# HpWang-whu/YOHO

Hardware: AMD Instinct MI355X
Metric: keypoints/sec (5000 kp x60 rot desc+YOHO-O) (higher is better)
Workload: dtype fp16x2 split (2^-22-accurate products, fp32 accumulate); 1 GPU

## Files before the change

yoho_amd/csrc/gemmf.h:

```cpp
#pragma once
#include <hip/hip_runtime.h>
#include <type_traits>
#include "common.h"

namespace yoho {

typedef float floatx16 __attribute__((ext_vector_type(16)));
typedef float floatx4 __attribute__((ext_vector_type(4)));
typedef unsigned uintx4 __attribute__((ext_vector_type(4)));
typedef _Float16 halfx8 __attribute__((ext_vector_type(8)));
typedef const __attribute__((address_space(1))) void* gptr_t;
typedef __attribute__((address_space(3))) void* lptr_t;

constexpr int FG_STAGE = 32768;
constexpr int FG_LDS = 4 * FG_STAGE;

static const int FG_ORD_D[NIR_ORD] = {5, 4, 3, 3, 1};
static const int FG_ORD_R[NIR_ORD] = {4, 3, 1, 2, 0};
static const int FG_IR_BASE[5] = {0, 1, 10, 19, 35};
static const int FG_IR_D[5] = {1, 3, 3, 4, 5};

struct FGemmArgs {
    const char* A;
    const char* B;
    const float* bias;
    const float* res;
    float* out;
    long long a_off[NIR_ORD], b_off[NIR_ORD];
    int NT[NIR_ORD], MT[NIR_ORD], rot[NIR_ORD];
    int dim[NIR_ORD], qbase[NIR_ORD];
    int cin, cout, kppad, nT32;
    float descale;
    int* rflag;
    const unsigned* amax;
};

template <int I, int N, typename Fn>
__device__ __forceinline__ void sfor(Fn&& f) {
    if constexpr (I < N) {
        f(std::integral_constant<int, I>{});
        sfor<I + 1, N>(f);
    }
}

__device__ __forceinline__ floatx16 mfma_h(uintx4 a, uintx4 b, floatx16 c) {
    union { uintx4 u; halfx8 h; } ca, cb;
    ca.u = a; cb.u = b;
    return __builtin_amdgcn_mfma_f32_32x32x16_f16(ca.h, cb.h, c, 0, 0, 0);
}

__device__ __forceinline__ const char* uniform_ptr(const char* p) {
    const unsigned long long v = reinterpret_cast<unsigned long long>(p);
    const unsigned lo = __builtin_amdgcn_readfirstlane((unsigned)v), hi = __builtin_amdgcn_readfirstlane((unsigned)(v >> 32));
    return reinterpret_cast<const char*>(((unsigned long long)hi << 32) | lo);
}

template <int MI, int NJ>
__device__ __forceinline__ void zero_acc(floatx16 (&acc)[MI][NJ]) {
#pragma unroll
    for (int i = 0; i < MI; ++i)
#pragma unroll
        for (int j = 0; j < NJ; ++j)
#pragma unroll
            for (int e = 0; e < 16; ++e) acc[i][j][e] = 0.f;
}

__device__ __forceinline__ bool fg3_map(const FGemmArgs& a, int xcd, int slot, int& t, int& local, int& r) {
    int start = 0;
    for (int u = 0; u < NIR_ORD; ++u) {
        const int ru = (xcd + a.rot[u]) & 7;
        const int cnt = a.NT[u] > ru ? ((a.NT[u] - 1 - ru) / 8 + 1) * a.MT[u] : 0;
        if (slot < start + cnt) { t = u; local = slot - start; r = ru; return true; }
        start += cnt;
    }
    return false;
}

inline int fgemm_grid(const FGemmArgs& a, int per_tile) {
    int tot = 0;
    for (int x = 0; x < 8; ++x) {
        int n = 0;
        for (int t = 0; t < NIR_ORD; ++t) {
            const int r = (x + a.rot[t]) & 7;
            if (a.NT[t] > r) n += ((a.NT[t] - 1 - r) / 8 + 1) * a.MT[t] * per_tile;
        }
        tot = n > tot ? n : tot;
    }
    return 8 * tot;
}

enum { F2_NOSTORE = 0x100, F2_MIX = 0x200, F2_ST_SC1 = 0x400, F2_ST_NT = 0x800, F2_SPARSE4 = 0x1000, F2_SPARSE16 = 0x2000 };

__device__ __forceinline__ size_t slab_off(int tile32, int q, int cout8, int o, int half, int kp32) {
    return (((((size_t)tile32 * G + q) * cout8 + (o >> 3)) * 2 + half) * TILE + kp32) * 4;
}

template <int MI, int NJ>
__device__ __forceinline__ void residual_start(floatx16 (&acc)[MI][NJ], int row0, int kp0, int jidx, int d, int qbase, const float* res, float descale,
                                               int cout, int nT32, int lane) {
    const float inv = 1.f / descale;
    const int half = lane >> 5, kp32 = lane & 31, cout8 = cout >> 3;
#pragma unroll
    for (int bi = 0; bi < NJ; ++bi) {
        const int tile32 = (kp0 >> 5) + bi;
#pragma unroll
        for (int ai = 0; ai < MI; ++ai) {
            const int rowb = row0 + ai * 32;
            const int iidx = rowb / cout, o0 = rowb - iidx * cout;
            const bool ok = tile32 < nT32 && iidx < d;
            const int q = qbase + iidx * d + jidx;
#pragma unroll
            for (int q4 = 0; q4 < 4; ++q4) {
                const size_t off = slab_off(tile32, q, cout8, o0 + q4 * 8 + half * 4, half, kp32);
                const floatx4 v = *reinterpret_cast<const floatx4*>(res + (ok ? off : 0)) * (ok ? inv : 0.f);
                acc[ai][bi][4 * q4 + 0] = v.x; acc[ai][bi][4 * q4 + 1] = v.y;
                acc[ai][bi][4 * q4 + 2] = v.z; acc[ai][bi][4 * q4 + 3] = v.w;
            }
        }
    }
}

template <int MI, int NJ>
__device__ __forceinline__ void coef_epilogue(const floatx16 (&acc)[MI][NJ], int row0, int kp0, int jidx, int d, int qbase, float* out, const float* bias,
                                              float descale, int cout, int nT32, int* rflag, int lane, int flags) {
    const int half = lane >> 5, kp32 = lane & 31, cout8 = cout >> 3;
    unsigned top = 0u;
#ifdef YOHO_EXPERIMENTS
    if ((flags & F2_SPARSE4) && (blockIdx.x >> 3) % 4 != 0) flags |= F2_NOSTORE;
    if ((flags & F2_SPARSE16) && (blockIdx.x >> 3) % 16 != 0) flags |= F2_NOSTORE;
    const __amdgpu_buffer_rsrc_t orsrc = __builtin_amdgcn_make_buffer_rsrc(out, 0, 0x7FFFFFFF, 0x00020000);
#endif
#pragma unroll
    for (int bi = 0; bi < NJ; ++bi) {
        const int tile32 = (kp0 >> 5) + bi;
        if (tile32 >= nT32) continue;
#pragma unroll
        for (int ai = 0; ai < MI; ++ai) {
            const int rowb = row0 + ai * 32;
            const int iidx = rowb / cout, o0 = rowb - iidx * cout;
            if (iidx >= d) continue;
            const int q = qbase + iidx * d + jidx;
#pragma unroll
            for (int q4 = 0; q4 < 4; ++q4) {
                const int o = o0 + q4 * 8 + half * 4;
                floatx4 val;
                val.x = acc[ai][bi][4 * q4 + 0]; val.y = acc[ai][bi][4 * q4 + 1];
                val.z = acc[ai][bi][4 * q4 + 2]; val.w = acc[ai][bi][4 * q4 + 3];
                val *= descale;
                if (d == 1) val += *reinterpret_cast<const floatx4*>(bias + o) * 7.745966692414834f;
                const size_t off = slab_off(tile32, q, cout8, o, half, kp32);
#ifdef YOHO_EXPERIMENTS
                if (flags & F2_ST_SC1) __builtin_amdgcn_raw_buffer_store_b128(__builtin_bit_cast(uintx4, val), orsrc, (int)(off * 4), 0, 16);
                else if (flags & F2_ST_NT) __builtin_amdgcn_raw_buffer_store_b128(__builtin_bit_cast(uintx4, val), orsrc, (int)(off * 4), 0, 2);
                else if (!(flags & F2_NOSTORE))
#endif
                *reinterpret_cast<floatx4*>(out + off) = val;
                top = max(max(top, __float_as_uint(val.x) & 0x7FFFFFFFu), __float_as_uint(val.y) & 0x7FFFFFFFu);
                top = max(max(top, __float_as_uint(val.z) & 0x7FFFFFFFu), __float_as_uint(val.w) & 0x7FFFFFFFu);
            }
        }
    }
    note_range_bits(rflag, top, FP16_MAX / HF_ASCALE);
}

void fgemm_fill_args(FGemmArgs& a, const Layer& L, const char* Bplanes, int kppad, int nT32, const float* res, float* out, int* rflag);
int launch_fgemm2(const FGemmArgs& a, int flags, hipStream_t s);
int launch_fgemm3(const FGemmArgs& a, int flags, hipStream_t s);
int fgemm2_init();

}
```

yoho_amd/csrc/gemmf.hip:

```cpp
#include <hip/hip_runtime.h>
#include <hip/hip_fp16.h>
#include <type_traits>
#include <vector>
#include <cmath>
#include <cstring>
#include <cstdlib>

#include "common.h"
#include "gemmf.h"

namespace yoho {

struct Frags {
    uintx4 ah[4], al[4], bh[4], bl[4];
};

template <int SUB, int R>
__device__ __forceinline__ void read_frag(const char* pa, const char* pb, Frags& f) {
    constexpr int t = R & 3;
    if constexpr (R < 4) f.al[t] = *reinterpret_cast<const uintx4*>(pa + (2 + SUB) * 8192 + t * 512);
    else if constexpr (R < 8) f.bh[t] = *reinterpret_cast<const uintx4*>(pb + (0 + SUB) * 8192 + t * 512);
    else if constexpr (R < 12) f.ah[t] = *reinterpret_cast<const uintx4*>(pa + (0 + SUB) * 8192 + t * 512);
    else f.bl[t] = *reinterpret_cast<const uintx4*>(pb + (2 + SUB) * 8192 + t * 512);
}
// ... 28 lines not shown
        acc[g >> 2][g & 3] = mfma_h(f.al[g >> 2], f.bh[g & 3], acc[g >> 2][g & 3]);
        read_frag<RSUB, g>(ra, rb, nf);
        __builtin_amdgcn_sched_barrier(0);
    });
    sfor<0, 16>([&](auto gc) {
        constexpr int g = decltype(gc)::value;
        acc[g >> 2][g & 3] = mfma_h(f.ah[g >> 2], f.bl[g & 3], acc[g >> 2][g & 3]);
        if constexpr (DMA) {
            stage_unit<g>(srcA, srcB, dmadst, w, lane16);
            __builtin_amdgcn_sched_barrier(0);
        }
    });
    __builtin_amdgcn_sched_barrier(0);
    sfor<0, 16>([&](auto gc) {
        constexpr int g = decltype(gc)::value;
        acc[g >> 2][g & 3] = mfma_h(f.ah[g >> 2], f.bh[g & 3], acc[g >> 2][g & 3]);
    });
    __builtin_amdgcn_sched_barrier(0);
}

__global__ __launch_bounds__(256, 1) void fgemm_kernel(FGemmArgs a, int flags) {
    extern __shared__ __attribute__((aligned(16))) char smem[];
    const int tid = threadIdx.x, lane = tid & 63;
    const int w = __builtin_amdgcn_readfirstlane(tid >> 6);
    int t = 0, local = 0, r = 0;
    if (!fg3_map(a, blockIdx.x & 7, blockIdx.x >> 3, t, local, r)) return;
    const int d = a.dim[t];
    const int MT = a.MT[t], KS = d * a.cin / 32;
    const int cg = local / MT, mtile = local - cg * MT;
    const int ntile = r + 8 * cg;
    const char* Ag = a.A + a.a_off[t] + (size_t)mtile * KS * FG_STAGE;
    const char* Bg = a.B + a.b_off[t] + (size_t)ntile * KS * FG_STAGE;
    const int wm = w >> 1, wn = w & 1;
    const int lane16 = lane * 16;
    const int row0 = mtile * 256 + wm * 128;
    const int col0 = ntile * 256 + wn * 128;

    floatx16 acc[4][4];
    zero_acc(acc);

    const int lane_a = (lane >> 5) * 4096 + (wm * 128 + (lane & 31)) * 16;
    const int lane_b = FG_STAGE + (lane >> 5) * 4096 + (wn * 128 + (lane & 31)) * 16;

    stage_tile(Ag, smem, w, lane);
    stage_tile(Bg, smem + FG_STAGE, w, lane);
    if (KS > 1) {
        stage_tile(Ag + FG_STAGE, smem + 2 * FG_STAGE, w, lane);
        stage_tile(Bg + FG_STAGE, smem + 3 * FG_STAGE, w, lane);
    }
    if ((flags & EPI_RES) && row0 < d * a.cout) residual_start(acc, row0, col0 % a.kppad, col0 / a.kppad, d, a.qbase[t], a.res, a.descale, a.cout, a.nT32, lane);
    asm volatile("s_waitcnt vmcnt(0)" ::: "memory");
    __syncthreads();

    if (row0 >= d * a.cout) {
        for (int s = 0; s < KS; ++s) {
            asm volatile("s_waitcnt vmcnt(0)" ::: "memory");
            __syncthreads();
            const int s2 = s + 2 < KS ? s + 2 : KS - 1;
            char* cur = smem + (s & 1) * (2 * FG_STAGE);
            stage_tile(Ag + (size_t)s2 * FG_STAGE, cur, w, lane);
            stage_tile(Bg + (size_t)s2 * FG_STAGE, cur + FG_STAGE, w, lane);
        }
        asm volatile("s_waitcnt vmcnt(0)" ::: "memory");
        return;
    }
    Frags P, Q;
    read_frags<0>(smem + lane_a, smem + lane_b, P);
    for (int s = 0; s < KS; ++s) {
        char* cur = smem + (s & 1) * (2 * FG_STAGE);
        char* nxt = smem + ((s + 1) & 1) * (2 * FG_STAGE);
        substep<1, false>(P, acc, cur + lane_a, cur + lane_b, Q, nullptr, nullptr, nullptr, w, lane16);
        asm volatile("s_waitcnt vmcnt(0) lgkmcnt(0)" ::: "memory");
        __syncthreads();
        __builtin_amdgcn_sched_barrier(0);
        const int s2 = s + 2 < KS ? s + 2 : KS - 1;
        substep<0, true>(Q, acc, nxt + lane_a, nxt + lane_b, P, uniform_ptr(Ag + (size_t)s2 * FG_STAGE), uniform_ptr(Bg + (size_t)s2 * FG_STAGE),
                              cur, w, lane16);
    }
    asm volatile("s_waitcnt vmcnt(0)" ::: "memory");

    coef_epilogue(acc, row0, col0 % a.kppad, col0 / a.kppad, d, a.qbase[t], a.out, a.bias, a.descale, a.cout, a.nT32, a.rflag, lane, flags);
}

int fgemm_init() {
    HIPCHK(hipFuncSetAttribute(reinterpret_cast<const void*>(&fgemm_kernel), hipFuncAttributeMaxDynamicSharedMemorySize, FG_LDS));
    if (int rc = cgemm_init()) return rc;
    return fgemm2_init();
}

static long long pack_off(int t, int rows, int kdim) {
    long long off = 0;
    for (int u = 0; u < t; ++u) off += (long long)((FG_ORD_D[u] * rows + 255) / 256) * (FG_ORD_D[u] * kdim / 32) * FG_STAGE;
    return off;
}

size_t fgemm_planes_bytes(int kppad, int cin) { return (size_t)pack_off(NIR_ORD, kppad, cin); }

void fgemm_qinfo(int* qi ) {
    for (int t = 0; t < NIR_ORD; ++t) {
        const int r = FG_ORD_R[t], d = FG_IR_D[r];
        for (int m = 0; m < d; ++m)
            for (int j = 0; j < d; ++j) {
                int* p = qi + (FG_IR_BASE[r] + m * d + j) * 4;
                p[0] = t; p[1] = m; p[2] = j; p[3] = d;
            }
    }
}
void fgemm_plane_offsets(int kppad, int cin, long long* off ) {
    for (int t = 0; t < NIR_ORD; ++t) off[t] = pack_off(t, kppad, cin);
}

static inline unsigned short half_bits_h(float x) {
    const _Float16 h = (_Float16)x;
    unsigned short u;
    std::memcpy(&u, &h, 2);
    return u;
}

static unsigned char e4m3_bits(float x) {
    const unsigned sgn = std::signbit(x) ? 0x80u : 0u;
    const float a = std::fabs(x);
    if (!(a == a)) return 0x7F;
    if (a >= 464.f) return (unsigned char)(sgn | 0x7E);
    if (a < std::ldexp(1.f, -6)) {
        const int r = (int)std::nearbyint(std::ldexp(a, 9));
        return (unsigned char)(sgn | (r == 8 ? 0x08 : r));
    }
    int e;
    (void)std::frexp(a, &e);
    int r = (int)std::nearbyint(std::ldexp(a, 3 - (e - 1)));
    if (r == 16) { r = 8; ++e; }
    const int E = e - 1 + 7;
    if (E > 15 || (E == 15 && r - 8 > 6)) return (unsigned char)(sgn | 0x7E);
    return (unsigned char)(sgn | (E << 3) | (r - 8));
}
static inline float half_value_h(unsigned short u) {
    _Float16 h;
    std::memcpy(&h, &u, 2);
    return (float)h;
}

static inline size_t apack_index(int row, int k, int KS) {
    const int mtile = row >> 8, rr = row & 255, ks = k >> 5, sub = (k >> 4) & 1, kg = (k >> 3) & 1, e = k & 7;
    return ((size_t)mtile * KS + ks) * (FG_STAGE / 2) + ((size_t)(sub * 2 + kg) * 256 + rr) * 8 + e;
}
static inline void put_split(unsigned short* pack, size_t idx, float x) {
    const _Float16 hi = (_Float16)x;
    pack[idx] = half_bits_h(x);
    pack[idx + 8192] = half_bits_h(x - (float)hi);
}
static void fp8_correction_planes(const std::vector<unsigned short>& out, std::vector<unsigned short>& out8) {
    out8 = out;
    const size_t nblk = out.size() / (FG_STAGE / 2);
    for (size_t b = 0; b < nblk; ++b) {
        const unsigned short* src = out.data() + b * (FG_STAGE / 2);
        unsigned char* dst = reinterpret_cast<unsigned char*>(out8.data() + b * (FG_STAGE / 2) + 8192);
        for (int u = 0; u < 1024; ++u)
            for (int e = 0; e < 8; ++e) {
                dst[u * 16 + e] = e4m3_bits(half_value_h(src[u * 8 + e]) * 0.25f);
                dst[u * 16 + 8 + e] = e4m3_bits(half_value_h(src[8192 + u * 8 + e]) * 512.f);
            }
    }
}

int pack_fgemm_weights(const FourierBasis& fb, const float* W, int cin, int cout, std::vector<unsigned short>& out, float* descale,
                       std::vector<unsigned short>* out8) {
    if ((cout % 256 && cout != 32) || cin % 32) return -1;
    std::vector<float> what((size_t)60 * cout * cin);
    std::vector<double> coef(60 * NTAP);
    for (int r = 0; r < 5; ++r) {
        const int d = FG_IR_D[r];
        for (int i = 0; i < d; ++i)
            for (int m = 0; m < d; ++m)
                for (int k = 0; k < NTAP; ++k) coef[(FG_IR_BASE[r] + i * d + m) * NTAP + k] = fb.rho[r][fb.n0[k]][m * d + i];
    }
    float wmax = 0.f;
    for (int f = 0; f < 60; ++f)
        for (int o = 0; o < cout; ++o)
            for (int c = 0; c < cin; ++c) {
                const float* wk = W + ((size_t)o * cin + c) * NTAP;
                double acc = 0.0;
                for (int k = 0; k < NTAP; ++k) acc += (double)wk[k] * coef[f * NTAP + k];
                const float v = (float)acc;
                what[((size_t)f * cout + o) * cin + c] = v;
                wmax = std::fmax(wmax, std::fabs(v));
            }
    int ex = 0;
    if (wmax > 0.f && std::isfinite(wmax)) (void)std::frexp(wmax, &ex);
    const float wscale = std::ldexp(1.f, 10 - ex);
    *descale = 1.f / (wscale * HF_ASCALE);
    out.assign((size_t)pack_off(NIR_ORD, cout, cin) / 2, 0);
    for (int t = 0; t < NIR_ORD; ++t) {
        const int r = FG_ORD_R[t], d = FG_IR_D[r];
        unsigned short* base = out.data() + pack_off(t, cout, cin) / 2;
        for (int i = 0; i < d; ++i)
            for (int o = 0; o < cout; ++o)
                for (int m = 0; m < d; ++m) {
                    const float* src = &what[((size_t)(FG_IR_BASE[r] + i * d + m) * cout + o) * cin];
                    for (int c = 0; c < cin; ++c) put_split(base, apack_index(i * cout + o, m * cin + c, d * cin / 32), src[c] * wscale);
                }
    }
    if (out8) fp8_correction_planes(out, *out8);
    return 0;
}

int pack_cgemm_weights(const float* W, int cin, int cout, int ntaps, std::vector<unsigned short>& out, float* descale, std::vector<unsigned short>& out8) {
    if (cout % 256 || cin % 32) return -1;
    float wmax = 0.f;
    for (size_t i = 0; i < (size_t)cout * cin * ntaps; ++i) wmax = std::fmax(wmax, std::fabs(W[i]));
    int ex = 0;
    if (wmax > 0.f && std::isfinite(wmax)) (void)std::frexp(wmax, &ex);
    const float wscale = std::ldexp(1.f, 10 - ex);
    *descale = 1.f / (wscale * H2_ASCALE);
    const int KS = ntaps * cin / 32;
    out.assign((size_t)(cout / 256) * KS * (FG_STAGE / 2), 0);
    for (int o = 0; o < cout; ++o)
        for (int tap = 0; tap < ntaps; ++tap)
            for (int c = 0; c < cin; ++c) put_split(out.data(), apack_index(o, tap * cin + c, KS), W[((size_t)o * cin + c) * ntaps + tap] * wscale);
    fp8_correction_planes(out, out8);
    return 0;
}

void fgemm_fill_args(FGemmArgs& a, const Layer& L, const char* Bplanes, int kppad, int nT32, const float* res, float* out, int* rflag) {
    a.rflag = rflag; a.amax = nullptr;
    a.A = reinterpret_cast<const char*>(L.wpg); a.B = Bplanes; a.bias = L.bias; a.res = res; a.out = out;
    a.cin = L.cin; a.cout = L.cout; a.kppad = kppad; a.nT32 = nT32; a.descale = L.wpg_descale;
    static const int ROT[NIR_ORD] = {0, 0, 4, 4, 2};
    for (int t = 0; t < NIR_ORD; ++t) {
        a.a_off[t] = pack_off(t, L.cout, L.cin);
        a.b_off[t] = pack_off(t, kppad, L.cin);
        a.MT[t] = (FG_ORD_D[t] * L.cout + 255) / 256;
        a.NT[t] = FG_ORD_D[t] * kppad / 256;
        a.rot[t] = ROT[t];
        a.dim[t] = FG_ORD_D[t];
        a.qbase[t] = FG_IR_BASE[FG_ORD_R[t]];
    }
}

int launch_fgemm(const Layer& L, const char* Bplanes, int kppad, int nT32, const float* res, float* out, int flags, hipStream_t s, int* rflag,
                 FGemmBlocking blocking, const unsigned* amax) {
    FGemmArgs a;
    fgemm_fill_args(a, L, Bplanes, kppad, nT32, res, out, rflag);
    static const int dbg_gemm1 = [] { const char* e = experiment_env("YOHO_PARTI_DEBUG"); return (e && std::strstr(e, "gemm1")) ? 1 : 0; }();
    if (dbg_gemm1) blocking = FG_TILE256_W4;
    if (blocking == FG_TILE256_W8 && amax && L.wpg8) { a.amax = amax; a.A = reinterpret_cast<const char*>(L.wpg8); }
    if (blocking == FG_TILE256_W8) return launch_fgemm3(a, flags, s);
    if (blocking != FG_TILE256_W4) return launch_fgemm2(a, flags, s);
    hipLaunchKernelGGL(fgemm_kernel, dim3(fgemm_grid(a, 1)), dim3(256), FG_LDS, s, a, flags);
    HIPCHK(hipGetLastError());
    return 0;
}

}
```

yoho_amd/csrc/gemmf2.hip:

```cpp
#include <hip/hip_runtime.h>
#include <cstdlib>
#include <cstring>
#include "common.h"
#include "gemmf.h"

namespace yoho {

constexpr int F2_BUF = 24576;
constexpr int F2_LDS = 3 * F2_BUF;
constexpr int F3_BUF = 32768;
constexpr int F3_LDS = 3 * F3_BUF;

struct Frags2 {
    uintx4 ah[4], al[4], bh[2], bl[2];
};

template <int LO, int R>
__device__ __forceinline__ void read_frag2(const char* pa, const char* pb, Frags2& f) {
    if constexpr (R < 4) f.al[R] = *reinterpret_cast<const uintx4*>(pa + 8192 + R * 512);
    else if constexpr (R < 6) f.bh[R - 4] = *reinterpret_cast<const uintx4*>(pb + (R - 4) * 512);
    else if constexpr (R < 10) f.ah[R - 6] = *reinterpret_cast<const uintx4*>(pa + (R - 6) * 512);
    else f.bl[R - 10] = *reinterpret_cast<const uintx4*>(pb + LO + (R - 10) * 512);
}
template <int LO>
// ... 135 lines not shown
    }
}

__global__ __launch_bounds__(256, 2) void fgemm2_kernel(FGemmArgs a, int flags) {
    extern __shared__ __attribute__((aligned(16))) char smem[];
    const int tid = threadIdx.x, lane = tid & 63;
    const int w = __builtin_amdgcn_readfirstlane(tid >> 6);
    int t = 0, local = 0, r = 0;
    if (!fg2_map(a, blockIdx.x & 7, blockIdx.x >> 3, (flags & F2_MIX) == 0, t, local, r)) return;
    const int d = a.dim[t];
    const int MT = a.MT[t], KS = d * a.cin / 32, KT = 2 * KS;
    const int nh = local & 1, pair = local >> 1;
    const int cg = pair / MT, mtile = pair - cg * MT;
    const int ntile = r + 8 * cg;
    const char* Ag = a.A + a.a_off[t] + (size_t)mtile * KS * FG_STAGE;
    const char* Bg = a.B + a.b_off[t] + (size_t)ntile * KS * FG_STAGE + nh * 2048;
    const int wm = w >> 1, wn = w & 1;
    const Dma2 dm(w, lane);
    const int lane_a = (lane >> 5) * 4096 + (wm * 128 + (lane & 31)) * 16;
    const int lane_b = 16384 + (lane >> 5) * 2048 + (wn * 64 + (lane & 31)) * 16;

    floatx16 acc[4][2];
    zero_acc(acc);
    auto dma = [&](int st, int buf) { dma_step(dm, Ag + step_off(st), Bg + step_off(st), smem + buf); };
    ring_prologue<F2_BUF>(KT, dma);
    const int row0 = mtile * 256 + wm * 128, colbase = ntile * 256 + nh * 128 + wn * 64;
    const bool rows_live = row0 < d * a.cout;
    const int jidx = colbase / a.kppad, kp0 = colbase - jidx * a.kppad, qbase = a.qbase[t];
    if ((flags & EPI_RES) && rows_live) residual_start(acc, row0, kp0, jidx, d, qbase, a.res, a.descale, a.cout, a.nT32, lane);
    asm volatile("s_waitcnt vmcnt(0)" ::: "memory");
    __builtin_amdgcn_s_barrier();
    if (!rows_live) return ring_pipelined_idle<F2_BUF>(KT, dma);

    Frags2 P;
    read_frags2<Dma2::LO>(smem + lane_a, smem + lane_b, P);
    ring_pipelined<F2_BUF, 6>(smem, Ag, Bg, KT, lane_a, lane_b, P,
        [&](auto dmac, const Frags2& f, Frags2& nf, const char* ra, const char* rb, const char* srcA, const char* srcB, char* buf) {
            step2<decltype(dmac)::value>(dm, f, acc, ra, rb, nf, srcA, srcB, buf);
        });
    coef_epilogue(acc, row0, kp0, jidx, d, qbase, a.out, a.bias, a.descale, a.cout, a.nT32, a.rflag, lane, flags);
}

struct Wave3 {
    int wm, wn, nh, lane_a, lane_b;
    Dma3 dm;
    __device__ __forceinline__ Wave3(int w8, int lane) : wm((w8 & 3) >> 1), wn(w8 & 1), nh(w8 >> 2), dm(w8, lane) {
        lane_a = (lane >> 5) * 4096 + (wm * 128 + (lane & 31)) * 16;
        lane_b = 16384 + (lane >> 5) * 4096 + (nh * 128 + wn * 64 + (lane & 31)) * 16;
    }
};

__global__ __launch_bounds__(512, 2) void fgemm3_kernel(FGemmArgs a, int flags) {
    extern __shared__ __attribute__((aligned(16))) char smem[];
    const int tid = threadIdx.x, lane = tid & 63;
    const Wave3 wv(__builtin_amdgcn_readfirstlane(tid >> 6), lane);
    int t = 0, local = 0, r = 0;
    if (!fg3_map(a, blockIdx.x & 7, blockIdx.x >> 3, t, local, r)) return;
    const int d = a.dim[t];
    const int MT = a.MT[t], KS = d * a.cin / 32, KT = 2 * KS;
    const int cg = local / MT, mtile = local - cg * MT;
    const int ntile = r + 8 * cg;
    const char* Ag = a.A + a.a_off[t] + (size_t)mtile * KS * FG_STAGE;
    const char* Bg = a.B + a.b_off[t] + (size_t)ntile * KS * FG_STAGE;

    floatx16 acc[4][2];
    zero_acc(acc);
    auto dma = [&](int st, int buf) { dma_step(wv.dm, Ag + step_off(st), Bg + step_off(st), smem + buf); };
    ring_prologue<F3_BUF>(KT, dma);
    const int row0 = mtile * 256 + wv.wm * 128, colbase = ntile * 256 + wv.nh * 128 + wv.wn * 64;
    const bool rows_live = row0 < d * a.cout;
    const int jidx = colbase / a.kppad, kp0 = colbase - jidx * a.kppad, qbase = a.qbase[t];
    if ((flags & EPI_RES) && rows_live) residual_start(acc, row0, kp0, jidx, d, qbase, a.res, a.descale, a.cout, a.nT32, lane);
    asm volatile("s_waitcnt vmcnt(0)" ::: "memory");
    __builtin_amdgcn_s_barrier();
    if (!rows_live) return ring_pipelined_idle<F3_BUF>(KT, dma);

    Frags2 P;
    read_frags2<Dma3::LO>(smem + wv.lane_a, smem + wv.lane_b, P);
    ring_pipelined<F3_BUF, 4>(smem, Ag, Bg, KT, wv.lane_a, wv.lane_b, P,
        [&](auto dmac, const Frags2& f, Frags2& nf, const char* ra, const char* rb, const char* srcA, const char* srcB, char* buf) {
            step2<decltype(dmac)::value>(wv.dm, f, acc, ra, rb, nf, srcA, srcB, buf);
        });
    coef_epilogue(acc, row0, kp0, jidx, d, qbase, a.out, a.bias, a.descale, a.cout, a.nT32, a.rflag, lane, flags);
}

typedef int intx8 __attribute__((ext_vector_type(8)));
typedef short shortx2 __attribute__((ext_vector_type(2)));
typedef _Float16 halfx2 __attribute__((ext_vector_type(2)));
struct Frags8 {
    intx8 a[4], b[2];
};
struct C8Scales {
    float ah = 4.f, al = 4.f / 2048.f, bh = 1.f, bl = 1.f;
    int mfma_b = 127;
    C8Scales() = default;
    __device__ __forceinline__ explicit C8Scales(const unsigned* amax) {
        const unsigned amax_bits = __builtin_amdgcn_readfirstlane(*amax);
        int kexp = (int)(amax_bits >> 23) - 127 - 7;
        kexp = kexp < -60 ? -60 : (kexp > 9 ? 9 : kexp);
        bh = __uint_as_float((unsigned)(kexp + 127) << 23); bl = __uint_as_float((unsigned)(kexp - 11 + 127) << 23);
        mfma_b = 127 + kexp;
    }
};
struct Int2 { int x, y; };
__device__ __forceinline__ Int2 frag_to_fp8(uintx4 f, float scale) {
    union { unsigned u; halfx2 h; } p0, p1, p2, p3;
    p0.u = f[0]; p1.u = f[1]; p2.u = f[2]; p3.u = f[3];
    shortx2 r = {0, 0}, q = {0, 0};
    r = __builtin_amdgcn_cvt_scalef32_pk_fp8_f16(r, p0.h, scale, false);
    r = __builtin_amdgcn_cvt_scalef32_pk_fp8_f16(r, p1.h, scale, true);
    q = __builtin_amdgcn_cvt_scalef32_pk_fp8_f16(q, p2.h, scale, false);
    q = __builtin_amdgcn_cvt_scalef32_pk_fp8_f16(q, p3.h, scale, true);
    Int2 o;
    __builtin_memcpy(&o.x, &r, 4);
    __builtin_memcpy(&o.y, &q, 4);
    return o;
}

template <int PAR>
__device__ __forceinline__ void step3c(const Frags2& f, floatx16 (&acc)[4][2], Frags8& c8, const C8Scales& sc) {
#pragma unroll
    for (int i = 0; i < 4; ++i)
#pragma unroll
        for (int j = 0; j < 2; ++j) acc[i][j] = mfma_h(f.ah[i], f.bh[j], acc[i][j]);
#pragma unroll
    for (int i = 0; i < 4; ++i)
#pragma unroll
        for (int e = 0; e < 4; ++e) c8.a[i][4 * PAR + e] = (int)f.al[i][e];
#pragma unroll
    for (int j = 0; j < 2; ++j) {
        const Int2 l = frag_to_fp8(f.bl[j], sc.bl), h = frag_to_fp8(f.bh[j], sc.bh);
        c8.b[j][4 * PAR] = l.x; c8.b[j][4 * PAR + 1] = l.y; c8.b[j][4 * PAR + 2] = h.x; c8.b[j][4 * PAR + 3] = h.y;
    }
    if constexpr (PAR == 1) {
#pragma unroll
        for (int i = 0; i < 4; ++i)
#pragma unroll
            for (int j = 0; j < 2; ++j)
                acc[i][j] = __builtin_amdgcn_mfma_scale_f32_32x32x64_f8f6f4(c8.a[i], c8.b[j], acc[i][j], 0, 0, 0, 127 + 2 - 11, 0, sc.mfma_b);
    }
}

template <bool FP8, typename BSrc>
__device__ __forceinline__ void ring_plain(floatx16 (&acc)[4][2], char* smem, const Wave3& wv, const char* Ag, BSrc&& bsrc, int KT, bool rows_live,
                                           const C8Scales& sc) {
    Frags8 c8;
    if constexpr (FP8) {
#pragma unroll
        for (int i = 0; i < 4; ++i)
#pragma unroll
            for (int e = 0; e < 8; ++e) c8.a[i][e] = 0;
#pragma unroll
        for (int j = 0; j < 2; ++j)
#pragma unroll
            for (int e = 0; e < 8; ++e) c8.b[j][e] = 0;
    }
    int cur = 0, stg = 2 * F3_BUF;
    int s = 0;
    auto stage = [&] {
        const int s2 = s + 2 < KT ? s + 2 : KT - 1;
        dma_step(wv.dm, uniform_ptr(Ag + step_off(s2)), uniform_ptr(bsrc(s2)), smem + stg);
    };
    auto rotate = [&] { stg = cur; cur = cur == 2 * F3_BUF ? 0 : cur + F3_BUF; ++s; };
    auto one_step = [&](auto parity) {
        asm volatile("s_waitcnt vmcnt(4) lgkmcnt(0)" ::: "memory");
        __builtin_amdgcn_s_barrier();
// ... 188 lines not shown

template <int R>
__device__ __forceinline__ void read_frag3s(const char* pa, const char* pb, Frags3s& f) {
    if constexpr (R < 5) f.al[R] = *reinterpret_cast<const uintx4*>(pa + 8192 + R * 512);
    else if constexpr (R == 5) f.bh = *reinterpret_cast<const uintx4*>(pb);
    else if constexpr (R < 11) f.ah[R - 6] = *reinterpret_cast<const uintx4*>(pa + (R - 6) * 512);
    else f.bl = *reinterpret_cast<const uintx4*>(pb + 8192);
}

template <bool DMA, int D>
__device__ __forceinline__ void step3s(const Frags3s& f, floatx16 (&acc)[5][1], const char* ra, const char* rb, Frags3s& nf,
                                       const char* srcA, const char* srcB, char* dmabuf, const Dma3& dm) {
    sfor<0, 5>([&](auto gc) {
        constexpr int g = decltype(gc)::value;
        if constexpr (g < D) acc[g][0] = mfma_h(f.al[g], f.bh, acc[g][0]);
        if constexpr (g < D) read_frag3s<g>(ra, rb, nf);
        if constexpr (g == 4) read_frag3s<5>(ra, rb, nf);
        __builtin_amdgcn_sched_barrier(0);
    });
    sfor<0, 5>([&](auto gc) {
        constexpr int g = decltype(gc)::value;
        if constexpr (g < D) acc[g][0] = mfma_h(f.ah[g], f.bl, acc[g][0]);
        if constexpr (g < D) read_frag3s<6 + g>(ra, rb, nf);
        if constexpr (g == 4) read_frag3s<11>(ra, rb, nf);
        __builtin_amdgcn_sched_barrier(0);
    });
    sfor<0, 5>([&](auto gc) {
        constexpr int g = decltype(gc)::value;
        if constexpr (g < D) acc[g][0] = mfma_h(f.ah[g], f.bh, acc[g][0]);
        if constexpr (DMA && g < 4) dm.template piece<g>(srcA, srcB, dmabuf);
        __builtin_amdgcn_sched_barrier(0);
    });
}

template <int D>
__device__ __forceinline__ void fgemm3s_kloop(floatx16 (&acc)[5][1], char* smem, const char* Ag, const char* Bg, int KT, const Dma3& dm, int lane_a, int lane_b) {
    Frags3s P;
    sfor<0, 12>([&](auto rc) {
        constexpr int R = decltype(rc)::value;
        if constexpr (R == 5 || R == 11 || (R < 5 && R < D) || (R > 5 && R < 11 && R - 6 < D)) read_frag3s<R>(smem + lane_a, smem + lane_b, P);
    });
    ring_pipelined<F3_BUF, 4>(smem, Ag, Bg, KT, lane_a, lane_b, P,
        [&](auto dmac, const Frags3s& f, Frags3s& nf, const char* ra, const char* rb, const char* srcA, const char* srcB, char* buf) {
            step3s<decltype(dmac)::value, D>(f, acc, ra, rb, nf, srcA, srcB, buf, dm);
        });
}

__global__ __launch_bounds__(512, 2) void fgemm3s_kernel(FGemmArgs a, int flags) {
    extern __shared__ __attribute__((aligned(16))) char smem[];
    const int tid = threadIdx.x, lane = tid & 63;
    const int w8 = __builtin_amdgcn_readfirstlane(tid >> 6);
    int t = 0, local = 0, r = 0;
    if (!fg3_map(a, blockIdx.x & 7, blockIdx.x >> 3, t, local, r)) return;
    const int d = a.dim[t];
    const int KS = d * a.cin / 32, KT = 2 * KS;
    const int ntile = r + 8 * local;
    const char* Ag = a.A + a.a_off[t];
    const char* Bg = a.B + a.b_off[t] + (size_t)ntile * KS * FG_STAGE;
    const Dma3 dm(w8, lane);
    const int lane_a = (lane >> 5) * 4096 + (lane & 31) * 16;
    const int lane_b = 16384 + (lane >> 5) * 4096 + (w8 * 32 + (lane & 31)) * 16;

    floatx16 acc[5][1];
    zero_acc(acc);
    ring_prologue<F3_BUF>(KT, [&](int st, int buf) { dma_step(dm, uniform_ptr(Ag + step_off(st)), uniform_ptr(Bg + step_off(st)), smem + buf); });
    asm volatile("s_waitcnt vmcnt(0)" ::: "memory");
    __builtin_amdgcn_s_barrier();

    switch (d) {
        case 1: fgemm3s_kloop<1>(acc, smem, Ag, Bg, KT, dm, lane_a, lane_b); break;
        case 3: fgemm3s_kloop<3>(acc, smem, Ag, Bg, KT, dm, lane_a, lane_b); break;
        case 4: fgemm3s_kloop<4>(acc, smem, Ag, Bg, KT, dm, lane_a, lane_b); break;
        default: fgemm3s_kloop<5>(acc, smem, Ag, Bg, KT, dm, lane_a, lane_b); break;
    }
    const int colbase = ntile * 256 + w8 * 32;
    const int jidx = colbase / a.kppad, kp0 = colbase - jidx * a.kppad;
    coef_epilogue(acc, 0, kp0, jidx, d, a.qbase[t], a.out, a.bias, a.descale, 32, a.nT32, a.rflag, lane, flags & F2_NOSTORE);
}

int fgemm3_init() {
    HIPCHK(hipFuncSetAttribute(reinterpret_cast<const void*>(&fgemm3_kernel), hipFuncAttributeMaxDynamicSharedMemorySize, F3_LDS));
    HIPCHK(hipFuncSetAttribute(reinterpret_cast<const void*>(&fgemm3s_kernel), hipFuncAttributeMaxDynamicSharedMemorySize, F3_LDS));
    HIPCHK(hipFuncSetAttribute(reinterpret_cast<const void*>(&fgemm3c_kernel), hipFuncAttributeMaxDynamicSharedMemorySize, F3_LDS));
    return 0;
}

int launch_fgemm3(const FGemmArgs& a, int flags, hipStream_t s) {
    if (const char* dbg = experiment_env("YOHO_FGEMM_DEBUG")) {
        if (std::strstr(dbg, "nostore")) flags |= F2_NOSTORE;
        if (std::strstr(dbg, "sc1")) flags |= F2_ST_SC1;
        if (std::strstr(dbg, "stnt")) flags |= F2_ST_NT;
    }
    const int tot = fgemm_grid(a, 1);
    static const bool small_ok = [] { const char* e = experiment_env("YOHO_FGEMM_DEBUG"); return !(e && std::strstr(e, "nosmall")); }();
    if (small_ok && a.cout == 32 && !(flags & EPI_RES)) hipLaunchKernelGGL(fgemm3s_kernel, dim3(tot), dim3(512), F3_LDS, s, a, flags);
    else if (a.amax) hipLaunchKernelGGL(fgemm3c_kernel, dim3(tot), dim3(512), F3_LDS, s, a, flags);
    else hipLaunchKernelGGL(fgemm3_kernel, dim3(tot), dim3(512), F3_LDS, s, a, flags);
    HIPCHK(hipGetLastError());
    return 0;
}

int fgemm2_init() {
    HIPCHK(hipFuncSetAttribute(reinterpret_cast<const void*>(&fgemm2_kernel), hipFuncAttributeMaxDynamicSharedMemorySize, F2_LDS));
    return fgemm3_init();
}

int launch_fgemm2(const FGemmArgs& a, int flags, hipStream_t s) {
    if (const char* dbg = experiment_env("YOHO_FGEMM_DEBUG")) {
        if (std::strstr(dbg, "nostore")) flags |= F2_NOSTORE;
        if (std::strstr(dbg, "mix")) flags |= F2_MIX;
        if (std::strstr(dbg, "sc1")) flags |= F2_ST_SC1;
        if (std::strstr(dbg, "nt")) flags |= F2_ST_NT;
        if (std::strstr(dbg, "sparse4")) flags |= F2_SPARSE4;
        if (std::strstr(dbg, "sparse16")) flags |= F2_SPARSE16;
    }
    hipLaunchKernelGGL(fgemm2_kernel, dim3(fgemm_grid(a, 2)), dim3(256), F2_LDS, s, a, flags);
    HIPCHK(hipGetLastError());
    return 0;
}

}
```

Before: 1.891 million keypoints/s.

## Add 16x16x32 MFMA GEMM kernel variants for wide layers

Adds new GEMM kernels for the three blocking schemes that use the 16x16x32 f16 MFMA instead of 32x32x16, with matching residual and epilogue routines that permute lanes back to the existing slab layout. They are selected automatically for layers with cin and cout of at least 256 when no fp8 amax path is active. The aim is higher MFMA throughput and different register and LDS reuse on large layers, at the cost of extra permlane swaps in the epilogue and more code paths to keep correct.

```diff
diff --git a/yoho_amd/csrc/gemmf.h b/yoho_amd/csrc/gemmf.h
--- a/yoho_amd/csrc/gemmf.h
+++ b/yoho_amd/csrc/gemmf.h
@@ -89,7 +89,7 @@
     return 8 * tot;
 }
 
-enum { F2_NOSTORE = 0x100, F2_MIX = 0x200, F2_ST_SC1 = 0x400, F2_ST_NT = 0x800, F2_SPARSE4 = 0x1000, F2_SPARSE16 = 0x2000 };
+enum { F2_NOSTORE = 0x100, F2_MIX = 0x200, F2_ST_SC1 = 0x400, F2_ST_NT = 0x800, F2_SPARSE4 = 0x1000, F2_SPARSE16 = 0x2000, F2_K32 = 0x4000 };
 
 __device__ __forceinline__ size_t slab_off(int tile32, int q, int cout8, int o, int half, int kp32) {
     return (((((size_t)tile32 * G + q) * cout8 + (o >> 3)) * 2 + half) * TILE + kp32) * 4;
@@ -163,6 +163,129 @@
     note_range_bits(rflag, top, FP16_MAX / HF_ASCALE);
 }
 
+__device__ __forceinline__ floatx4 mfma_h16(uintx4 a, uintx4 b, floatx4 c) {
+    union { uintx4 u; halfx8 h; } ca, cb;
+    ca.u = a; cb.u = b;
+    return __builtin_amdgcn_mfma_f32_16x16x32_f16(ca.h, cb.h, c, 0, 0, 0);
+}
+
+inline bool fgemm_layer_k32(const FGemmArgs& a) { return a.cin >= 256 && a.cin % 64 == 0 && a.cout >= 256; }
+
+template <int NJ, typename Extra>
+__device__ __forceinline__ void row_products32(floatx4 (&accrow)[NJ], const uintx4& al, const uintx4& ah, const uintx4 (&bh)[NJ], const uintx4 (&bl)[NJ],
+                                               Extra&& extra) {
+    sfor<0, 3 * NJ>([&](auto mc) {
+        constexpr int m = decltype(mc)::value, j = m % NJ, p = m / NJ;
+        accrow[j] = mfma_h16(p == 0 ? al : ah, p == 1 ? bl[j] : bh[j], accrow[j]);
+        __builtin_amdgcn_sched_barrier(0);
+        extra(mc);
+        __builtin_amdgcn_sched_barrier(0);
+    });
+}
+
+template <int LOB, int MI, int NJ>
+__device__ __forceinline__ void stage32_plain(floatx4 (&acc)[MI][NJ], const char* pa, const char* pb) {
+    uintx4 bh[NJ], bl[NJ], al[2], ah[2];
+#pragma unroll
+    for (int j = 0; j < NJ; ++j) {
+        bh[j] = *reinterpret_cast<const uintx4*>(pb + j * 256);
+        bl[j] = *reinterpret_cast<const uintx4*>(pb + LOB + j * 256);
+    }
+    al[0] = *reinterpret_cast<const uintx4*>(pa + 16384);
+    ah[0] = *reinterpret_cast<const uintx4*>(pa);
+    sfor<0, MI>([&](auto ic) {
+        constexpr int i = decltype(ic)::value;
+        if constexpr (i + 1 < MI) {
+            al[(i + 1) & 1] = *reinterpret_cast<const uintx4*>(pa + 16384 + (i + 1) * 256);
+            ah[(i + 1) & 1] = *reinterpret_cast<const uintx4*>(pa + (i + 1) * 256);
+        }
+        row_products32(acc[i], al[i & 1], ah[i & 1], bh, bl, [](auto) {});
+    });
+}
+
+template <int MI, int NJ>
+__device__ __forceinline__ void zero_acc(floatx4 (&acc)[MI][NJ]) {
+#pragma unroll
+    for (int i = 0; i < MI; ++i)
+#pragma unroll
+        for (int j = 0; j < NJ; ++j) acc[i][j] = floatx4{0.f, 0.f, 0.f, 0.f};
+}
+
+template <bool TO_SLAB>
+__device__ __forceinline__ void swap_rows16(floatx4& x, floatx4& y) {
+    typedef unsigned uintx2 __attribute__((ext_vector_type(2)));
+#pragma unroll
+    for (int e = 0; e < 4; ++e) {
+        uintx2 r = {__float_as_uint(x[e]), __float_as_uint(y[e])};
+        if constexpr (TO_SLAB) {
+            r = __builtin_amdgcn_permlane16_swap(r.x, r.y, false, false);
+            r = __builtin_amdgcn_permlane32_swap(r.x, r.y, false, false);
+        } else {
+            r = __builtin_amdgcn_permlane32_swap(r.x, r.y, false, false);
+            r = __builtin_amdgcn_permlane16_swap(r.x, r.y, false, false);
+        }
+        x[e] = __uint_as_float(r.x); y[e] = __uint_as_float(r.y);
+    }
+}
+
+template <int MI, int NJ>
+__device__ __forceinline__ void residual_start(floatx4 (&acc)[MI][NJ], int row0, int kp0, int jidx, int d, int qbase, const float* res, float descale,
+                                               int cout, int nT32, int lane) {
+    static_assert(NJ % 2 == 0, "pairs of 16-column tiles");
+    const float inv = 1.f / descale;
+    const int half = lane >> 5, kp32 = lane & 31, cout8 = cout >> 3;
+#pragma unroll
+    for (int bi = 0; bi < NJ; bi += 2) {
+        const int tile32 = (kp0 >> 5) + (bi >> 1);
+#pragma unroll
+        for (int ai = 0; ai < MI; ++ai) {
+            const int rowb = row0 + ai * 16;
+            const int iidx = rowb / cout, o0 = rowb - iidx * cout;
+            const bool ok = tile32 < nT32 && iidx < d;
+            const int q = qbase + iidx * d + jidx;
+            const size_t off0 = slab_off(tile32, q, cout8, o0 + half * 4, half, kp32), off1 = slab_off(tile32, q, cout8, o0 + 8 + half * 4, half, kp32);
+            acc[ai][bi] = *reinterpret_cast<const floatx4*>(res + (ok ? off0 : 0)) * (ok ? inv : 0.f);
+            acc[ai][bi + 1] = *reinterpret_cast<const floatx4*>(res + (ok ? off1 : 0)) * (ok ? inv : 0.f);
+            swap_rows16<false>(acc[ai][bi], acc[ai][bi + 1]);
+        }
+    }
+}
+
+template <int MI, int NJ>
+__device__ __forceinline__ void coef_epilogue(const floatx4 (&acc)[MI][NJ], int row0, int kp0, int jidx, int d, int qbase, float* out, const float* bias,
+                                              float descale, int cout, int nT32, int* rflag, int lane, int flags) {
+    static_assert(NJ % 2 == 0, "pairs of 16-column tiles");
+    const int half = lane >> 5, kp32 = lane & 31, cout8 = cout >> 3;
+    unsigned top = 0u;
+#pragma unroll
+    for (int bi = 0; bi < NJ; bi += 2) {
+        const int tile32 = (kp0 >> 5) + (bi >> 1);
+        if (tile32 >= nT32) continue;
+#pragma unroll
+        for (int ai = 0; ai < MI; ++ai) {
+            const int rowb = row0 + ai * 16;
+            const int iidx = rowb / cout, o0 = rowb - iidx * cout;
+            if (iidx >= d) continue;
+            const int q = qbase + iidx * d + jidx;
+            floatx4 v[2] = {acc[ai][bi], acc[ai][bi + 1]};
+            swap_rows16<true>(v[0], v[1]);
+#pragma unroll
+            for (int h8 = 0; h8 < 2; ++h8) {
+                const int o = o0 + h8 * 8 + half * 4;
+                floatx4 val = v[h8] * descale;
+                if (d == 1) val += *reinterpret_cast<const floatx4*>(bias + o) * 7.745966692414834f;
+#ifdef YOHO_EXPERIMENTS
+                if (!(flags & F2_NOSTORE))
+#endif
+                *reinterpret_cast<floatx4*>(out + slab_off(tile32, q, cout8, o, half, kp32)) = val;
+                top = max(max(top, __float_as_uint(val.x) & 0x7FFFFFFFu), __float_as_uint(val.y) & 0x7FFFFFFFu);
+                top = max(max(top, __float_as_uint(val.z) & 0x7FFFFFFFu), __float_as_uint(val.w) & 0x7FFFFFFFu);
+            }
+        }
+    }
+    note_range_bits(rflag, top, FP16_MAX / HF_ASCALE);
+}
+
 void fgemm_fill_args(FGemmArgs& a, const Layer& L, const char* Bplanes, int kppad, int nT32, const float* res, float* out, int* rflag);
 int launch_fgemm2(const FGemmArgs& a, int flags, hipStream_t s);
 int launch_fgemm3(const FGemmArgs& a, int flags, hipStream_t s);
diff --git a/yoho_amd/csrc/gemmf.hip b/yoho_amd/csrc/gemmf.hip
--- a/yoho_amd/csrc/gemmf.hip
+++ b/yoho_amd/csrc/gemmf.hip
@@ -134,8 +134,52 @@
     coef_epilogue(acc, row0, col0 % a.kppad, col0 / a.kppad, d, a.qbase[t], a.out, a.bias, a.descale, a.cout, a.nT32, a.rflag, lane, flags);
 }
 
+__global__ __launch_bounds__(256, 1) void fgemmk_kernel(FGemmArgs a, int flags) {
+    extern __shared__ __attribute__((aligned(16))) char smem[];
+    const int tid = threadIdx.x, lane = tid & 63;
+    const int w = __builtin_amdgcn_readfirstlane(tid >> 6);
+    int t = 0, local = 0, r = 0;
+    if (!fg3_map(a, blockIdx.x & 7, blockIdx.x >> 3, t, local, r)) return;
+    const int d = a.dim[t];
+    const int MT = a.MT[t], KS = d * a.cin / 32;
+    const int cg = local / MT, mtile = local - cg * MT;
+    const int ntile = r + 8 * cg;
+    const char* Ag = a.A + a.a_off[t] + (size_t)mtile * KS * FG_STAGE;
+    const char* Bg = a.B + a.b_off[t] + (size_t)ntile * KS * FG_STAGE;
+    const int wm = w >> 1, wn = w & 1;
+    const int row0 = mtile * 256 + wm * 128, col0 = ntile * 256 + wn * 128;
+    const bool rows_live = row0 < d * a.cout;
+    const int lane_a = (lane >> 4) * 4096 + (wm * 128 + (lane & 15)) * 16;
+    const int lane_b = FG_STAGE + (lane >> 4) * 4096 + (wn * 128 + (lane & 15)) * 16;
+
+    floatx4 acc[8][8];
+    zero_acc(acc);
+    stage_tile(Ag, smem, w, lane);
+    stage_tile(Bg, smem + FG_STAGE, w, lane);
+    if (KS > 1) {
+        stage_tile(Ag + FG_STAGE, smem + 2 * FG_STAGE, w, lane);
+        stage_tile(Bg + FG_STAGE, smem + 3 * FG_STAGE, w, lane);
+    }
+    if ((flags & EPI_RES) && rows_live) residual_start(acc, row0, col0 % a.kppad, col0 / a.kppad, d, a.qbase[t], a.res, a.descale, a.cout, a.nT32, lane);
+    asm volatile("s_waitcnt vmcnt(0)" ::: "memory");
+    __syncthreads();
+    for (int s = 0; s < KS; ++s) {
+        char* cur = smem + (s & 1) * (2 * FG_STAGE);
+        if (rows_live) stage32_plain<FG_STAGE / 2>(acc, cur + lane_a, cur + lane_b);
+        asm volatile("s_waitcnt vmcnt(0) lgkmcnt(0)" ::: "memory");
+        __syncthreads();
+        __builtin_amdgcn_sched_barrier(0);
+        if (s + 2 < KS) {
+            stage_tile(uniform_ptr(Ag + (size_t)(s + 2) * FG_STAGE), cur, w, lane);
+            stage_tile(uniform_ptr(Bg + (size_t)(s + 2) * FG_STAGE), cur + FG_STAGE, w, lane);
+        }
+    }
+    if (rows_live) coef_epilogue(acc, row0, col0 % a.kppad, col0 / a.kppad, d, a.qbase[t], a.out, a.bias, a.descale, a.cout, a.nT32, a.rflag, lane, flags);
+}
+
 int fgemm_init() {
     HIPCHK(hipFuncSetAttribute(reinterpret_cast<const void*>(&fgemm_kernel), hipFuncAttributeMaxDynamicSharedMemorySize, FG_LDS));
+    HIPCHK(hipFuncSetAttribute(reinterpret_cast<const void*>(&fgemmk_kernel), hipFuncAttributeMaxDynamicSharedMemorySize, FG_LDS));
     if (int rc = cgemm_init()) return rc;
     return fgemm2_init();
 }
@@ -296,9 +340,12 @@
     static const int dbg_gemm1 = [] { const char* e = experiment_env("YOHO_PARTI_DEBUG"); return (e && std::strstr(e, "gemm1")) ? 1 : 0; }();
     if (dbg_gemm1) blocking = FG_TILE256_W4;
     if (blocking == FG_TILE256_W8 && amax && L.wpg8) { a.amax = amax; a.A = reinterpret_cast<const char*>(L.wpg8); }
+    const char* dbg = experiment_env("YOHO_FGEMM_DEBUG");
+    if (fgemm_layer_k32(a) && !a.amax && !(dbg && std::strstr(dbg, "k16"))) flags |= F2_K32;
     if (blocking == FG_TILE256_W8) return launch_fgemm3(a, flags, s);
     if (blocking != FG_TILE256_W4) return launch_fgemm2(a, flags, s);
-    hipLaunchKernelGGL(fgemm_kernel, dim3(fgemm_grid(a, 1)), dim3(256), FG_LDS, s, a, flags);
+    if (flags & F2_K32) hipLaunchKernelGGL(fgemmk_kernel, dim3(fgemm_grid(a, 1)), dim3(256), FG_LDS, s, a, flags);
+    else hipLaunchKernelGGL(fgemm_kernel, dim3(fgemm_grid(a, 1)), dim3(256), FG_LDS, s, a, flags);
     HIPCHK(hipGetLastError());
     return 0;
 }
diff --git a/yoho_amd/csrc/gemmf2.hip b/yoho_amd/csrc/gemmf2.hip
--- a/yoho_amd/csrc/gemmf2.hip
+++ b/yoho_amd/csrc/gemmf2.hip
@@ -241,6 +241,173 @@
             step2<decltype(dmac)::value>(wv.dm, f, acc, ra, rb, nf, srcA, srcB, buf);
         });
     coef_epilogue(acc, row0, kp0, jidx, d, qbase, a.out, a.bias, a.descale, a.cout, a.nT32, a.rflag, lane, flags);
+}
+
+constexpr int F3K_BUF = 2 * FG_STAGE;
+constexpr int F3K_LDS = 2 * F3K_BUF;
+
+struct Dma3k {
+    static constexpr int NP = 8;
+    int la, ldst;
+    __device__ __forceinline__ Dma3k(int w8, int lane) : la(w8 * 1024 + lane * 16), ldst(w8 * 1024) {}
+    template <int U>
+    __device__ __forceinline__ void piece(const char* srcA, const char* srcB, char* buf) const {
+        constexpr int q = (U & 3) * 8192;
+        if constexpr (U < 4) __builtin_amdgcn_global_load_lds((gptr_t)(srcA + q + la), (lptr_t)(buf + q + ldst), 16, 0, 0);
+        else __builtin_amdgcn_global_load_lds((gptr_t)(srcB + q + la), (lptr_t)(buf + FG_STAGE + q + ldst), 16, 0, 0);
+    }
+};
+struct FragsA32 { uintx4 al, ah; };
+struct FragsB32 { uintx4 bh[4], bl[4]; };
+
+template <int R>
+__device__ __forceinline__ void read_open32(const char* pa, const char* pb, FragsA32& a0, FragsB32& b) {
+    if constexpr (R == 0) a0.al = *reinterpret_cast<const uintx4*>(pa + 16384);
+    else if constexpr (R < 5) b.bh[R - 1] = *reinterpret_cast<const uintx4*>(pb + (R - 1) * 256);
+    else if constexpr (R == 5) a0.ah = *reinterpret_cast<const uintx4*>(pa);
+    else b.bl[R - 6] = *reinterpret_cast<const uintx4*>(pb + 16384 + (R - 6) * 256);
+}
+
+template <bool DMA>
+__device__ __forceinline__ void step32(const Dma3k& dm, floatx4 (&acc)[8][4], FragsA32 (&fa)[2], const FragsB32& b, FragsB32& nb, const char* pa,
+                                       const char* npa, const char* npb, const char* srcA, const char* srcB, char* dmabuf) {
+    sfor<0, 7>([&](auto ic) {
+        constexpr int i = decltype(ic)::value;
+        row_products32(acc[i], fa[i & 1].al, fa[i & 1].ah, b.bh, b.bl, [&](auto mc) {
+            constexpr int m = decltype(mc)::value;
+            if constexpr (m == 1) fa[(i + 1) & 1].al = *reinterpret_cast<const uintx4*>(pa + 16384 + (i + 1) * 256);
+            if constexpr (m == 2) fa[(i + 1) & 1].ah = *reinterpret_cast<const uintx4*>(pa + (i + 1) * 256);
+        });
+    });
+    asm volatile("s_waitcnt vmcnt(0) lgkmcnt(0)" ::: "memory");
+    __builtin_amdgcn_s_barrier();
+    __builtin_amdgcn_sched_barrier(0);
+    row_products32(acc[7], fa[1].al, fa[1].ah, b.bh, b.bl, [&](auto mc) {
+        constexpr int m = decltype(mc)::value;
+        if constexpr (m < 5) {
+            read_open32<2 * m>(npa, npb, fa[0], nb);
+            read_open32<2 * m + 1>(npa, npb, fa[0], nb);
+        }
+        if constexpr (DMA && m >= 4) dm.template piece<m - 4>(srcA, srcB, dmabuf);
+    });
+}
+
+__global__ __launch_bounds__(512, 2) void fgemm3k_kernel(FGemmArgs a, int flags) {
+    extern __shared__ __attribute__((aligned(16))) char smem[];
+    const int tid = threadIdx.x, lane = tid & 63;
+    const int w8 = __builtin_amdgcn_readfirstlane(tid >> 6);
+    int t = 0, local = 0, r = 0;
+    if (!fg3_map(a, blockIdx.x & 7, blockIdx.x >> 3, t, local, r)) return;
+    const int d = a.dim[t];
+    const int MT = a.MT[t], KS = d * a.cin / 32;
+    const int cg = local / MT, mtile = local - cg * MT;
+    const int ntile = r + 8 * cg;
+    const char* Ag = a.A + a.a_off[t] + (size_t)mtile * KS * FG_STAGE;
+    const char* Bg = a.B + a.b_off[t] + (size_t)ntile * KS * FG_STAGE;
+    const int wm = (w8 & 3) >> 1, wn = w8 & 1, nh = w8 >> 2;
+    const Dma3k dm(w8, lane);
+    const int lane_a = (lane >> 4) * 4096 + (wm * 128 + (lane & 15)) * 16;
+    const int lane_b = FG_STAGE + (lane >> 4) * 4096 + (nh * 128 + wn * 64 + (lane & 15)) * 16;
+
+    floatx4 acc[8][4];
+    zero_acc(acc);
+    auto dma = [&](int st, int buf) {
+        const char* sa = uniform_ptr(Ag + (size_t)st * FG_STAGE);
+        const char* sb = uniform_ptr(Bg + (size_t)st * FG_STAGE);
+        sfor<0, Dma3k::NP>([&](auto uc) { dm.template piece<decltype(uc)::value>(sa, sb, smem + buf); });
+    };
+    dma(0, 0);
+    if (KS > 1) dma(1, F3K_BUF);
+    const int row0 = mtile * 256 + wm * 128, colbase = ntile * 256 + nh * 128 + wn * 64;
+    const bool rows_live = row0 < d * a.cout;
+    const int jidx = colbase / a.kppad, kp0 = colbase - jidx * a.kppad, qbase = a.qbase[t];
+    if ((flags & EPI_RES) && rows_live) residual_start(acc, row0, kp0, jidx, d, qbase, a.res, a.descale, a.cout, a.nT32, lane);
+    asm volatile("s_waitcnt vmcnt(0)" ::: "memory");
+    __builtin_amdgcn_s_barrier();
+    if (!rows_live) {
+        for (int s = 0; s < KS; ++s) {
+            asm volatile("s_waitcnt vmcnt(0)" ::: "memory");
+            __builtin_amdgcn_s_barrier();
+            if (s + 2 < KS) dma(s + 2, (s & 1) * F3K_BUF);
+        }
+        asm volatile("s_waitcnt vmcnt(0)" ::: "memory");
+        return;
+    }
+
+    FragsA32 fa[2];
+    FragsB32 P, Q;
+    sfor<0, 10>([&](auto rc) { read_open32<decltype(rc)::value>(smem + lane_a, smem + lane_b, fa[0], P); });
+    int s = 0, cur = 0;
+    auto run = [&](auto dmac, const FragsB32& b, FragsB32& nb) {
+        const int nxt = cur ^ F3K_BUF;
+        if constexpr (decltype(dmac)::value)
+            step32<true>(dm, acc, fa, b, nb, smem + cur + lane_a, smem + nxt + lane_a, smem + nxt + lane_b, uniform_ptr(Ag + (size_t)(s + 2) * FG_STAGE),
+                         uniform_ptr(Bg + (size_t)(s + 2) * FG_STAGE), smem + cur);
+        else
+            step32<false>(dm, acc, fa, b, nb, smem + cur + lane_a, smem + nxt + lane_a, smem + nxt + lane_b, nullptr, nullptr, nullptr);
+        cur = nxt; ++s;
+    };
+    constexpr std::true_type dmay;
+    constexpr std::false_type dman;
+    while (s + 2 < KS) {
+        run(dmay, P, Q);
+        run(dmay, Q, P);
+    }
+    run(dman, P, Q);
+    run(dman, Q, P);
+    coef_epilogue(acc, row0, kp0, jidx, d, qbase, a.out, a.bias, a.descale, a.cout, a.nT32, a.rflag, lane, flags);
+}
+
+constexpr int F2K_BUF = FG_STAGE + FG_STAGE / 2;
+constexpr int F2K_LDS = 2 * F2K_BUF;
+
+__global__ __launch_bounds__(256, 1) void fgemm2k_kernel(FGemmArgs a, int flags) {
+    extern __shared__ __attribute__((aligned(16))) char smem[];
+    const int tid = threadIdx.x, lane = tid & 63;
+    const int w = __builtin_amdgcn_readfirstlane(tid >> 6);
+    int t = 0, local = 0, r = 0;
+    if (!fg2_map(a, blockIdx.x & 7, blockIdx.x >> 3, (flags & F2_MIX) == 0, t, local, r)) return;
+    const int d = a.dim[t];
+    const int MT = a.MT[t], KS = d * a.cin / 32;
+    const int nh = local & 1, pair = local >> 1;
+    const int cg = pair / MT, mtile = pair - cg * MT;
+    const int ntile = r + 8 * cg;
+    const char* Ag = a.A + a.a_off[t] + (size_t)mtile * KS * FG_STAGE;
+    const char* Bg = a.B + a.b_off[t] + (size_t)ntile * KS * FG_STAGE + nh * 2048;
+    const int wm = w >> 1, wn = w & 1;
+    const int lane_a = (lane >> 4) * 4096 + (wm * 128 + (lane & 15)) * 16;
+    const int lane_b = FG_STAGE + (lane >> 4) * 2048 + (wn * 64 + (lane & 15)) * 16;
+
+    floatx4 acc[8][4];
+    zero_acc(acc);
+    auto dma = [&](int st, int buf) {
+        const char* sa = uniform_ptr(Ag + (size_t)st * FG_STAGE) + lane * 16;
+        const char* sb = uniform_ptr(Bg + (size_t)st * FG_STAGE) + lane * 16;
+#pragma unroll
+        for (int k = 0; k < 8; ++k) __builtin_amdgcn_global_load_lds((gptr_t)(sa + (k * 4 + w) * 1024), (lptr_t)(smem + buf + (k * 4 + w) * 1024), 16, 0, 0);
+#pragma unroll
+        for (int k = 0; k < 4; ++k) {
+            const int pb = w * 4 + k, u = pb >> 1, part = pb & 1;
+            __builtin_amdgcn_global_load_lds((gptr_t)(sb + u * 4096 + part * 1024), (lptr_t)(smem + buf + FG_STAGE + u * 2048 + part * 1024), 16, 0, 0);
+        }
+    };
+    dma(0, 0);
+    if (KS > 1) dma(1, F2K_BUF);
+    const int row0 = mtile * 256 + wm * 128, colbase = ntile * 256 + nh * 128 + wn * 64;
+    const bool rows_live = row0 < d * a.cout;
+    const int jidx = colbase / a.kppad, kp0 = colbase - jidx * a.kppad, qbase = a.qbase[t];
+    if ((flags & EPI_RES) && rows_live) residual_start(acc, row0, kp0, jidx, d, qbase, a.res, a.descale, a.cout, a.nT32, lane);
+    asm volatile("s_waitcnt vmcnt(0)" ::: "memory");
+    __builtin_amdgcn_s_barrier();
+    for (int s = 0; s < KS; ++s) {
+        const int cur = (s & 1) * F2K_BUF;
+        if (rows_live) stage32_plain<FG_STAGE / 4>(acc, smem + cur + lane_a, smem + cur + lane_b);
+        asm volatile("s_waitcnt vmcnt(0) lgkmcnt(0)" ::: "memory");
+        __builtin_amdgcn_s_barrier();
+        __builtin_amdgcn_sched_barrier(0);
+        if (s + 2 < KS) dma(s + 2, cur);
+    }
+    if (rows_live) coef_epilogue(acc, row0, kp0, jidx, d, qbase, a.out, a.bias, a.descale, a.cout, a.nT32, a.rflag, lane, flags);
 }
 
 typedef int intx8 __attribute__((ext_vector_type(8)));
@@ -595,6 +762,7 @@
     HIPCHK(hipFuncSetAttribute(reinterpret_cast<const void*>(&fgemm3_kernel), hipFuncAttributeMaxDynamicSharedMemorySize, F3_LDS));
     HIPCHK(hipFuncSetAttribute(reinterpret_cast<const void*>(&fgemm3s_kernel), hipFuncAttributeMaxDynamicSharedMemorySize, F3_LDS));
     HIPCHK(hipFuncSetAttribute(reinterpret_cast<const void*>(&fgemm3c_kernel), hipFuncAttributeMaxDynamicSharedMemorySize, F3_LDS));
+    HIPCHK(hipFuncSetAttribute(reinterpret_cast<const void*>(&fgemm3k_kernel), hipFuncAttributeMaxDynamicSharedMemorySize, F3K_LDS));
     return 0;
 }
 
@@ -608,6 +776,7 @@
     static const bool small_ok = [] { const char* e = experiment_env("YOHO_FGEMM_DEBUG"); return !(e && std::strstr(e, "nosmall")); }();
     if (small_ok && a.cout == 32 && !(flags & EPI_RES)) hipLaunchKernelGGL(fgemm3s_kernel, dim3(tot), dim3(512), F3_LDS, s, a, flags);
     else if (a.amax) hipLaunchKernelGGL(fgemm3c_kernel, dim3(tot), dim3(512), F3_LDS, s, a, flags);
+    else if (flags & F2_K32) hipLaunchKernelGGL(fgemm3k_kernel, dim3(tot), dim3(512), F3K_LDS, s, a, flags);
     else hipLaunchKernelGGL(fgemm3_kernel, dim3(tot), dim3(512), F3_LDS, s, a, flags);
     HIPCHK(hipGetLastError());
     return 0;
@@ -615,6 +784,7 @@
 
 int fgemm2_init() {
     HIPCHK(hipFuncSetAttribute(reinterpret_cast<const void*>(&fgemm2_kernel), hipFuncAttributeMaxDynamicSharedMemorySize, F2_LDS));
+    HIPCHK(hipFuncSetAttribute(reinterpret_cast<const void*>(&fgemm2k_kernel), hipFuncAttributeMaxDynamicSharedMemorySize, F2K_LDS));
     return fgemm3_init();
 }
 
@@ -627,7 +797,8 @@
         if (std::strstr(dbg, "sparse4")) flags |= F2_SPARSE4;
         if (std::strstr(dbg, "sparse16")) flags |= F2_SPARSE16;
     }
-    hipLaunchKernelGGL(fgemm2_kernel, dim3(fgemm_grid(a, 2)), dim3(256), F2_LDS, s, a, flags);
+    if (flags & F2_K32) hipLaunchKernelGGL(fgemm2k_kernel, dim3(fgemm_grid(a, 2)), dim3(256), F2K_LDS, s, a, flags);
+    else hipLaunchKernelGGL(fgemm2_kernel, dim3(fgemm_grid(a, 2)), dim3(256), F2_LDS, s, a, flags);
     HIPCHK(hipGetLastError());
     return 0;
 }
```

Result: faster. 1.926 million keypoints/s, median of 6 (+1.9%).
